# GuildOfWeavers/distaff

Hardware: AMD Instinct MI355X
Metric: trace_cells_per_sec (higher is better)
Workload: dtype u128 (prime field 2^128-45*2^40+1, 4x u32 limbs)

## Files before the change

distaff_amd/csrc/ctx.h:

```cpp
#pragma once
#include <hip/hip_runtime.h>
#include <stdint.h>
#include <string.h>
#include <memory>
#include <string>
#include <map>
#include <vector>
#include "fe.h"
#include "../../include/distaff_hip.h"

struct __attribute__((aligned(16))) digest { uint32_t w[8]; };
#define AIR_PERIODIC_STRIDE 29

#ifndef NTT_TW4_PAIRS
#define NTT_TW4_PAIRS 0
#endif
#if NTT_TW4_PAIRS
typedef fe_tw tw4_t;
#else
typedef fe tw4_t;
#endif

#define DST_MAX_FRI_LAYERS 24

struct dst_switch_def { const char* name; bool product; const char* values; const char* what; };
static const dst_switch_def DST_SWITCHES[] = {
    {"DISTAFF_SHARD_DEBUG",        true,  "1",               "stderr line per tree exchange on rank 0; communicators record the order of their collectives (dst_comm_trace)"},
    {"DISTAFF_SHARD_TREE_GATHER",  true,  "1",               "sharded Merkle trees: all-gather of all boundary nodes + upper levels repeated on every rank (BASELINE north_star's all-gather-only form) instead of the k-range all-to-all"},
    {"DISTAFF_SHARD_NO_OVERLAP",   true,  "1",               "sharded prover: every collective on the context's main stream (no second stream / events) also on a stream-ordered transport"},
    {"DISTAFF_COMM_TIMEOUT_S",     true,  "seconds",         "communicators: limit of every host wait behind a collective (default 60; <= 0: none); on expiry the rank aborts the communicator and returns DST_ERR_COMM (dst_comm_set_timeout changes it per handle)"},
    {"DISTAFF_LOCAL_TRANSPORT",    true,  "blocking",        "in-process transport (dst_comm_init_local, dst_prove_sharded_local): drain every rank's stream around each collective instead of the stream-ordered form (events between the ranks' streams, nothing waited for)"},
    {"DISTAFF_TMP_REGS",           true,  "4..W",            "registers per transform launch = size of the staging array (default: as many as 12 GiB hold, at most W)"},
    {"DISTAFF_AIR",                false, "small|deep|generic", "force a more general constraint-kernel instance set than the trace shape needs (generic = per-operation formulation)"},
    {"DISTAFF_BOUNDARY",           false, "eval",            "boundary combinations by evaluation on the 8n domain (the reference's route) instead of coefficient form"},
    {"DISTAFF_COMBINE",            false, "steps",           "combine_polys / DEEP composition as the reference's sequence of whole-array steps instead of the fused passes"},
    {"DISTAFF_NTT",                false, "pre|3pass|reg|lds", "force a transform plan family"},
    {"DISTAFF_NTT_SHAPE",          false, "a,b",             "three-pass plans: log2 of the first two pass lengths"},
    {"DISTAFF_NTT_ORDER",          false, "0",               "first pass of an extension in coset-slow block order"},
    {"DISTAFF_NTT_WAVES",          false, "4|8",             "force the 512- or 1024-lane instances of the LDS passes"},
    {"DISTAFF_NTT_FIXED",          false, "0",               "use the any-shape instances where a shape-compiled one exists"},
    {"DISTAFF_NTT_DIF",            false, "0|1|2",           "first pass of an extension: coset DIT (0), pre-scale + DIF (1), DIT with last-stage twiddles from global memory (2)"},
    {"DISTAFF_NTT_DEBUG",          false, "1",               "print the occupancy of every transform launch shape once"},
    {"DISTAFF_LDE_BATCH",          false, "cols,cosets",     "registers x cosets per transform launch"},
    {"DISTAFF_FOLD8_DFT",          false, "0",               "8n-coefficient extensions without the fused fold + 8-point step"},
    {"DISTAFF_TRACE_BUFFER",       false, "1",               "give the trace its own buffer instead of coset 0 of the extension"},
    {"DISTAFF_MERKLE_LEVEL2_LOG",  false, "k",               "build two tree levels per launch from 2^k grandparents per launch on (default 2^19)"},
    {"DISTAFF_MERKLE_LEVELS",      false, "1",               "one launch per tree level"},
    {"DISTAFF_SYN_DIV_TABLES",     false, "1",               "synthetic division by power tables + scan instead of the blocked form"},
    {"DISTAFF_FRI_TAIL",           false, "0",               "no single-launch tail: every FRI layer by its own launches (the tail otherwise starts at the first layer of at most 2^13 elements)"},
    {"DISTAFF_FRI_CHAIN",          false, "0",               "FRI commit phase with a root read-back and a host draw per layer"},
    {"DISTAFF_FRI_REPLICATE_LOG",  false, "k",               "sharded prover: replicate FRI layers from 2^k elements on (default 2^17)"},
    {"DISTAFF_SHARD_FORCE_OVERLAP", false, "1",              "sharded prover: the two-stream choreography of a stream-ordered transport over a blocking one"},
    {"DISTAFF_TEST_STALL_COLLECTIVE", false, "k|k@r",        "communicators: fault injection -- before device collective number k (of rank r only) a kernel holds the stream until the communicator is aborted"},
};
enum : size_t {
    HS_WEIGHTS = 0,
    HS_WEIGHTS_BYTES = (4 * 128 + 4) * 16,
    HS_DEEP = 32768,
    HS_DEEP_HALF = 2048,
    HS_FRI_ROOTS = 40960,
    HS_FRI_SLOTS = 45056,
    HS_FRI_SLOT_BYTES = 800,
    HS_AIR_FLAG = 65536 - 64,
    HS_DRAWS = 65536,
    HS_DRAWS_BYTES = (344 + 160) * 16,
    HS_COMPOSE = 65536 + 8192,
    HS_COMPOSE_BYTES = 516 * 16,
    HS_STATUS = 65536 + 8192 + 8320,
    HS_STATUS_SLOTS = 32,
// ... 22 lines not shown
    DST_BUF_TRACE_LEAVES = 2,
    DST_BUF_TRACE_NODES = 3,
    DST_BUF_CEVAL_I = 4,
    DST_BUF_CEVAL_F = 5,
    DST_BUF_CEVAL_T = 6,
    DST_BUF_CPOLY = 7,
    DST_BUF_CEVALS = 8,
    DST_BUF_CNODES = 9,
    DST_BUF_COMP_POLY = 10,
    DST_BUF_COMP_EVALS = 11,
    DST_BUF_FRI_EVALS = 12,
    DST_BUF_FRI_NODES = 13,
    DST_BUF_FRI_LEAVES = 14,
};

struct NttInstance;
struct NttRegInstance;
enum NttKind : uint32_t { NTT_FIRST, NTT_MIDDLE, NTT_LAST };
struct NttPass {
    NttKind kind = NTT_FIRST;
    uint32_t log_len = 0;
    uint32_t log_tile = 0, pre = 0;
    uint32_t dit = 0;
    size_t lds = 0;
    const NttInstance* inst = nullptr;
    const NttRegInstance* reg = nullptr;
    const fe_tw* stage_tw[2] = {nullptr, nullptr}; const fe_tw* pre_tw[2] = {nullptr, nullptr}; const tw4_t* tw4[2] = {nullptr, nullptr};
};
struct NttPlan {
    uint32_t log_n1 = 0, log_n2 = 0;
    uint32_t log_n3 = 0;
    uint32_t count = 0;
    bool coset_slow = false; uint32_t debug = 0;
    NttPass pass[3], first_lde;
    const NttPass& at(uint32_t i, bool lde) const { return (i == 0 && lde) ? first_lde : pass[i]; }
};

struct dst_ctx {
    dst_params prm{};
    std::string err;
    std::map<std::string, std::string> sw_values;
    const char* sw(const char* name) const { auto it = sw_values.find(name); return it == sw_values.end() ? nullptr : it->second.c_str(); }
    bool sw_is(const char* name, const char* value) const { const char* v = sw(name); return v && !strcmp(v, value); }
    bool sw_flag(const char* name) const { const char* v = sw(name); return v && v[0] && v[0] != '0'; }
    void read_switches() {
        sw_values.clear();
        for (const dst_switch_def& d : DST_SWITCHES)
            if (d.product || DST_TEST_HOOKS) if (const char* v = getenv(d.name)) sw_values[d.name] = v;
    }
    int device = 0;
    hipStream_t stream = nullptr;

    uint32_t log_n = 0, log_b = 0, log_N = 0;
    size_t n = 0, B = 0, N = 0, W = 0;
    size_t Bc = 0, j0 = 0;
    size_t stack_depth = 0;
    NttPlan plan;
    std::vector<fe> air_draws;
    std::shared_ptr<void> open_plan;
    std::vector<uint64_t> open_plan_positions;
    uint8_t open_plan_root[32] = {0};
    int fri_rep_from = 0;
    bool fri_tail_pending = false;
    fe* fri_nat0 = nullptr;
    bool sharded_layout = false;

// ... 171 lines not shown
```

distaff_amd/csrc/kernels_ntt.hip:

```cpp
#include "ctx.h"
#include "host/ctx_tables.h"
#include <mutex>
#include <type_traits>
#include "ntt_lds.h"

#if defined(NTT_NO_ROTATE)
#define NTT_NO_ROTATE_DEFINED 1
#else
#define NTT_NO_ROTATE_DEFINED 0
#endif
#define NTT_TILE_ELEMS 4096

struct NttArgs {
    const fe* src; fe* dst;
    size_t src_col_stride, src_coset_stride;
    size_t dst_col_stride, dst_coset_stride;
    const fe_tw* stage_tw;
    const fe_tw* prescale;
    const fe_tw* dit_last;
    const tw4_t* tw4;
    size_t tw4_coset_stride;
    uint32_t log_n1, log_n2, tile , log_N, log_b;
    uint32_t j0;
    uint32_t has_scale;
    uint32_t tiles_per_block;
    uint32_t debug;
    size_t src_row_stride, dst_k_stride, src_batch_stride, dst_batch_stride;
    uint32_t batch_log;
    uint32_t dit;
    uint32_t groups, cosets, cols;
    uint32_t coset_fast;
    uint32_t pre;
    const fe_tw* pre_tw;
    fe_tw scale;
};

__device__ __forceinline__ fe load_fe(const fe* p) { return *p; }

__device__ __forceinline__ fe dom_pow(const fe* lo, const fe* hi, uint32_t lo_bits, uint64_t e) {
    uint32_t l = (uint32_t)e & ((1u << lo_bits) - 1u), h = (uint32_t)(e >> lo_bits);
    fe a = lo[l];
    if (h == 0) return a;
    return fe_mul(a, hi[h]);
}

__device__ __forceinline__ void ntt_block(const NttArgs& a, uint32_t& group, uint32_t& jl, uint32_t& col) {
    const uint32_t b = blockIdx.x, units = a.groups * a.cosets;
    uint32_t u;
    if (a.coset_fast) {
        const uint32_t s = b >> 3, pairs = a.cosets * a.cols, pair = s % pairs;
        group = (s / pairs) * 8u + (b & 7u);
        const uint32_t chunk = pair / (4u * a.cosets), in_chunk = pair - chunk * 4u * a.cosets;
        const uint32_t width = (chunk * 4u + 4u <= a.cols) ? 4u : a.cols - chunk * 4u;
        col = chunk * 4u + in_chunk % width; jl = in_chunk / width;
// ... 42 lines not shown
#if defined(NTT_LAB_STAMPS)
#define NTT_LAB_WG_STRIDE 61u
__device__ unsigned long long ntt_lab_buf[2 * 256 * 16 * 2 * 16];
extern "C" __attribute__((visibility("default"))) int dst_lab_stamps(unsigned long long* out, size_t count, int clear) {
    if (count > sizeof(ntt_lab_buf) / 8) return -1;
    if (hipMemcpyFromSymbol(out, HIP_SYMBOL(ntt_lab_buf), count * 8) != hipSuccess) return -2;
    if (clear) { static unsigned long long zero[2 * 256 * 16 * 2 * 16]; if (hipMemcpyToSymbol(HIP_SYMBOL(ntt_lab_buf), zero, sizeof zero) != hipSuccess) return -3; }
    return 0;
}
#define NTT_LAB_FLUSH(pass, it, st, nst) do { \
    if ((blockIdx.x % NTT_LAB_WG_STRIDE) == 0u && blockIdx.x / NTT_LAB_WG_STRIDE < 256u && (it) < 2u && (threadIdx.x & 63u) == 0u) { \
        unsigned long long* o_ = ntt_lab_buf + ((((size_t)(pass) * 256u + blockIdx.x / NTT_LAB_WG_STRIDE) * 16u + (threadIdx.x >> 6)) * 2u + (it)) * 16u; \
        for (int k_ = 0; k_ < (nst); k_++) o_[k_] = (st)[k_]; } } while (0)
#else
#define NTT_LAB_FLUSH(pass, it, st, nst) ((void)0)
#endif
extern __shared__ __attribute__((aligned(16))) unsigned char ntt_smem[];

template <int THREADS, int WPE = 4, bool PREFETCH = true, int LOG_LEN = 0, int LOG_T = 0, int PRE = 0>
__global__ void __launch_bounds__(THREADS, WPE) ntt_pass_a(NttArgs a, const fe* __restrict__ src_base, fe* __restrict__ dst_base) {
    constexpr int EPT = NTT_TILE_ELEMS / THREADS;
    fe* L = reinterpret_cast<fe*>(ntt_smem);
    const uint32_t log_n1 = LOG_LEN ? (uint32_t)LOG_LEN : a.log_n1;
    const uint32_t log_t = LOG_T ? (uint32_t)LOG_T : a.tile, T = 1u << log_t, n1 = 1u << log_n1;
    fe_tw* TW = reinterpret_cast<fe_tw*>(L + n1 * T);
    uint32_t group, jl, col;
    ntt_block(a, group, jl, col);
    uint32_t hh = 0;
    if (PRE) { const uint32_t half = a.groups >> 1; hh = group >= half ? 1u : 0u; group -= hh * half; }
    const uint32_t jg = a.j0 + jl;
    const fe* __restrict__ src0 = src_base + (size_t)col * a.src_col_stride + (size_t)jl * a.src_coset_stride;
    fe* __restrict__ dst0 = dst_base + (size_t)col * a.dst_col_stride + (size_t)jl * a.dst_coset_stride;
    const uint32_t pmask = (1u << (a.log_b + log_n1 + PRE)) - 1u;
    const uint32_t jv = jg + (hh << a.log_b);
    if (a.dit) {
        const uint32_t in_lds = a.dit_last ? n1 / 2 : n1;
        for (uint32_t i = threadIdx.x; i + 1 < in_lds; i += THREADS) {
            const uint32_t lb = 31u - (uint32_t)__clz(i + 1), k = i + 1 - (1u << lb);
            TW[i] = a.prescale[((jv + (k << (a.log_b + PRE))) << (log_n1 - lb - 1)) & pmask];
        }
    } else
    for (uint32_t i = threadIdx.x; i < n1 / 2; i += THREADS) TW[dif_tw_slot(i)] = a.stage_tw[i];
    const bool scaled = !a.dit && a.prescale != nullptr && jg != 0;
    fe pre0 = fe_zero(), pre1 = fe_zero(), pre2 = fe_zero(), pre3 = fe_zero(), pre4 = fe_zero(), pre5 = fe_zero(), pre6 = fe_zero(), pre7 = fe_zero();
    const uint32_t count = n1 * T;
#define NTT_EACH(M) { M(0, pre0) M(1, pre1) M(2, pre2) M(3, pre3) M(4, pre4) M(5, pre5) M(6, pre6) M(7, pre7) }
    const bool rot_a = a.dit && log_t == 2 && !NTT_NO_ROTATE_DEFINED;
#define NTT_COL_A(idx) (rot_a ? (((idx) + ((idx) >> log_t)) & (T - 1)) : ((idx) & (T - 1)))
    const fe_tw pre_c = (PRE && a.dit) ? a.prescale[(jg << log_n1) & pmask] : fe_tw{};
    auto pre_stage_a = [&](const fe& x0, const fe& x1, uint32_t row) -> fe {
        if (a.dit) { const fe t = fe_mul_tw(x1, pre_c); return hh ? fe_sub(x0, t) : fe_add(x0, t); }
        return hh ? fe_mul_tw(fe_sub(x0, x1), a.pre_tw[row]) : fe_add(x0, x1);
    };
#define NTT_FETCH_A1(e, var) if constexpr ((e) < EPT) { uint32_t idx = lane + (e) * THREADS; idx = idx < count ? idx : 0u; \
        if constexpr (PRE != 0) { const uint32_t row_ = idx >> log_t; const fe x0_ = src[NTT_LAB_SRC(row_, NTT_COL_A(idx), (row_ << a.log_n2) + NTT_COL_A(idx))], x1_ = src[NTT_LAB_SRC(row_ + 512u, NTT_COL_A(idx), ((row_ + n1) << a.log_n2) + NTT_COL_A(idx))]; var = pre_stage_a(x0_, x1_, row_); } \
        else var = src[NTT_LAB_SRC(idx >> log_t, NTT_COL_A(idx), ((idx >> log_t) << a.log_n2) + NTT_COL_A(idx))]; }
#define NTT_FETCH_A(tile) { const fe* __restrict__ src = src0 + (tile) * T; NTT_EACH(NTT_FETCH_A1) }
    const tw4_t* __restrict__ tw4 = a.tw4 + (size_t)jl * a.tw4_coset_stride;
    const uint32_t tile0 = group * a.tiles_per_block;
    uint32_t lane = threadIdx.x;
    if (PREFETCH) NTT_FETCH_A(tile0)
    for (uint32_t it = 0; it < a.tiles_per_block; it++) {
        const uint32_t tile = tile0 + it;
        unsigned long long st[16]; (void)st;
        NTT_STAMP_REAL(st, 14);
        NTT_STAMP(st, 8);
        lane = lds_opaque_lane();
        if (!PREFETCH) NTT_FETCH_A(tile)
        NTT_STAMP(st, 9);
        __syncthreads();
        NTT_STAMP(st, 10);
#define NTT_PUT_A(e, var) if constexpr ((e) < EPT) { const uint32_t idx = lane + (e) * THREADS; if (idx < count) { if (a.dit) L[lds_slot(__brev(idx >> log_t) >> (32 - log_n1), NTT_COL_A(idx), log_t)] = var; else L[lds_slot(idx >> log_t, idx & (T - 1), log_t)] = scaled ? fe_mul_tw(var, a.prescale[(jg * (idx >> log_t)) & pmask]) : var; } }
        NTT_EACH(NTT_PUT_A)
#undef NTT_PUT_A
        NTT_STAMP(st, 11);
        __syncthreads();
        NTT_STAMP(st, 12);
        if (PREFETCH && it + 1 < a.tiles_per_block) NTT_FETCH_A(tile + 1)
        if constexpr (LOG_LEN != 0) {
            if (a.dit) lds_ntt_dit_fixed<THREADS, LOG_LEN, LOG_T>(L, TW, a.dit_last ? a.dit_last + (size_t)((jg << PRE) + hh) * (n1 / 2) : nullptr, NttKeepInLds(), st);
            else lds_ntt_dif_fixed<THREADS, LOG_LEN, LOG_T>(L, TW, NttKeepInLds(), st);
        } else {
            if (a.dit) lds_ntt_dit<THREADS>(L, TW, log_n1, log_t, 1u, log_n1 + 1u, a.dit_last ? a.dit_last + (size_t)((jg << PRE) + hh) * (n1 / 2) : nullptr);
            else lds_ntt_dif<THREADS>(L, TW, log_n1, log_t, 1u, log_n1 + 1u);
        }
        constexpr int RB = WPE > 4 ? 1 : THREADS == 512 ? 2 : 4;
#if defined(NTT_LAB_DST_DENSE)
        fe* __restrict__ dst = dst_base + ((size_t)blockIdx.x * a.tiles_per_block + it) * count;
#else
        fe* __restrict__ dst = dst0 + tile * T;
#endif
        const tw4_t* __restrict__ tw = tw4 + tile * T;
        for (uint32_t base = 0; base < count; base += RB * THREADS) {
            fe v[RB]; tw4_t w[RB]; uint32_t off[RB]; bool ok[RB];
            static_for<0, RB>([&](auto q_) {
                constexpr int q = decltype(q_)::value;
                uint32_t idx = base + q * THREADS + lane;
                ok[q] = idx < count;
                idx = ok[q] ? idx : 0u;
                const uint32_t t = idx & (T - 1), r = idx >> log_t;
                const uint32_t k1 = ((a.dit ? r : __brev(r) >> (32 - log_n1)) << PRE) + hh;
                off[q] = (k1 << a.log_n2) + t;
                v[q] = L[idx];
                w[q] = tw[NTT_LAB_TW(r, t, off[q])];
#if defined(NTT_LAB_DST_DENSE)
                off[q] = idx;
#endif
            });
            static_for<0, RB>([&](auto q_) {
                constexpr int q = decltype(q_)::value;
#if NTT_TW4_PAIRS
                const fe out_q = fe_mul_tw(v[q], w[q]);
#else
                const fe out_q = fe_mul(v[q], w[q]);
#endif
#if NTT_STREAM_STORE
                if (ok[q]) fe_store_stream(dst + off[q], out_q);
#else
                if (ok[q]) dst[off[q]] = out_q;
#endif
            });
        }
        NTT_STAMP(st, 13);
        NTT_STAMP_REAL(st, 15);
        NTT_LAB_FLUSH(0, it, st, 16);
    }
}

template <int THREADS, int WPE = 4, bool PREFETCH = true, int LOG_LEN = 0, int LOG_T = 0, int PRE = 0>
__global__ void __launch_bounds__(THREADS, WPE) ntt_pass_b(NttArgs a, const fe* __restrict__ src_base, fe* __restrict__ dst_base) {
    constexpr int EPT = NTT_TILE_ELEMS / THREADS;
    fe* L = reinterpret_cast<fe*>(ntt_smem);
    const uint32_t log_n2 = LOG_LEN ? (uint32_t)LOG_LEN : a.log_n2;
    const uint32_t log_t = LOG_T ? (uint32_t)LOG_T : a.tile, T = 1u << log_t, n2 = 1u << log_n2;
    fe_tw* TW = reinterpret_cast<fe_tw*>(L + n2 * T);
    uint32_t g, jl, col;
    ntt_block(a, g, jl, col);
    uint32_t hh = 0;
    if (PRE) { const uint32_t half = a.groups >> 1; hh = g >= half ? 1u : 0u; g -= hh * half; }
    const uint32_t batch = g & ((1u << a.batch_log) - 1u), group = g >> a.batch_log;
    const fe* __restrict__ src = src_base + (size_t)col * a.src_col_stride + (size_t)jl * a.src_coset_stride + (size_t)batch * a.src_batch_stride;
    fe* __restrict__ dst = dst_base + (size_t)col * a.dst_col_stride + (size_t)jl * a.dst_coset_stride + (size_t)batch * a.dst_batch_stride;
    for (uint32_t i = threadIdx.x; i < n2 / 2; i += THREADS) TW[dif_tw_slot(i)] = a.stage_tw[i];
    fe pre0 = fe_zero(), pre1 = fe_zero(), pre2 = fe_zero(), pre3 = fe_zero(), pre4 = fe_zero(), pre5 = fe_zero(), pre6 = fe_zero(), pre7 = fe_zero();
    const uint32_t count = n2 * T;
    const bool colfast_b = log_t == 2 && !NTT_NO_ROTATE_DEFINED;
#define NTT_ROW_B(idx) (colfast_b ? ((idx) & (T - 1)) : ((idx) >> log_n2))
#define NTT_M2_B(idx) (colfast_b ? ((idx) >> log_t) : ((idx) & (n2 - 1)))
#if NTT_STREAM_B_LOAD
#define NTT_LOAD_B(p) fe_load_stream(p)
#else
#define NTT_LOAD_B(p) (*(p))
#endif
#define NTT_FETCH_B1(e, var) if constexpr ((e) < EPT) { uint32_t idx = lane + (e) * THREADS; idx = idx < count ? idx : 0u; \
        if constexpr (PRE != 0) { const uint32_t m_ = NTT_M2_B(idx); const fe* p_ = srct + NTT_ROW_B(idx) * row_stride + m_; const fe x0_ = p_[0], x1_ = p_[n2]; \
                                  var = hh ? fe_mul_tw(fe_sub(x0_, x1_), a.pre_tw[m_]) : fe_add(x0_, x1_); } \
        else var = NTT_LOAD_B(srct + (NTT_ROW_B(idx) * row_stride + NTT_M2_B(idx))); }
#define NTT_FETCH_B(tile) { const fe* __restrict__ srct = src + (size_t)((tile) * T) * a.src_row_stride; NTT_EACH(NTT_FETCH_B1) }
    const uint32_t row_stride = (uint32_t)a.src_row_stride;
    const uint32_t tile0 = group * a.tiles_per_block;
    uint32_t lane = threadIdx.x;
    if (PREFETCH) NTT_FETCH_B(tile0)
    for (uint32_t it = 0; it < a.tiles_per_block; it++) {
        const uint32_t k1_0 = (tile0 + it) * T;
        unsigned long long st[16]; (void)st;
        NTT_STAMP_REAL(st, 14);
        NTT_STAMP(st, 8);
        lane = lds_opaque_lane();
        if (!PREFETCH) NTT_FETCH_B(tile0 + it)
        NTT_STAMP(st, 9);
        __syncthreads();
        NTT_STAMP(st, 10);
#define NTT_PUT_B(e, var) if constexpr ((e) < EPT) { const uint32_t idx = lane + (e) * THREADS; if (idx < count) L[lds_slot(NTT_M2_B(idx), NTT_ROW_B(idx), log_t)] = var; }
        NTT_EACH(NTT_PUT_B)
#undef NTT_PUT_B
        NTT_STAMP(st, 11);
        __syncthreads();
        NTT_STAMP(st, 12);
        if (PREFETCH && it + 1 < a.tiles_per_block) NTT_FETCH_B(tile0 + it + 1)
        const OutB out{dst + k1_0, (uint32_t)a.dst_k_stride, log_n2, a.has_scale != 0, a.scale, (uint32_t)PRE, hh};
        const fe_tw* Wuse = TW;
        if constexpr (LOG_LEN != 0) lds_ntt_dif_fixed<THREADS, LOG_LEN, LOG_T, OutB>(L, Wuse, out, st);
        else lds_ntt_dif<THREADS, OutB>(L, Wuse, log_n2, log_t, 1u, log_n2 + 1u, out);
        NTT_STAMP(st, 13);
        NTT_STAMP_REAL(st, 15);
        NTT_LAB_FLUSH(1, it, st, 16);
    }
}

template <int LOGL> struct NttDigits;
template <> struct NttDigits<6>  { static constexpr int r1 = 3, r2 = 3, r3 = 0, log_t = 2; };
// ... 129 lines not shown
                fe v = x[u * R + rho];
                if (a.tw_lo != nullptr) {
                    uint64_t e = ((uint64_t)m2 * (((uint64_t)k << a.log_b) + (a.coset_twiddle ? jg : 0u))) & nmask;
                    if (e != 0) {
                        const uint32_t el = (uint32_t)e & ((1u << a.lo_bits) - 1u), eh = (uint32_t)(e >> a.lo_bits);
                        v = fe_mul_call(v, a.tw_lo[el]);
                        if (eh != 0) v = fe_mul_call(v, a.tw_hi[eh]);
                    }
                }
                if (a.has_scale) v = fe_mul_call(v, a.scale);
                dst[(size_t)k * a.out_stride_k + t] = v;
            });
        });
    }
}

struct NttInstance { bool pass_b; int threads, wpe; bool prefetch; int log_len, log_t, pre; void (*kernel)(NttArgs, const fe*, fe*); };
#define NTT_INSTANCE(PASS_B, KERNEL, ...) {PASS_B, __VA_ARGS__, KERNEL<__VA_ARGS__>}
static const NttInstance NTT_INSTANCES[] = {
    NTT_INSTANCE(false, ntt_pass_a, 512, 4, true, 0, 0, 0),  NTT_INSTANCE(true, ntt_pass_b, 512, 4, true, 0, 0, 0),
    NTT_INSTANCE(false, ntt_pass_a, 1024, 4, true, 0, 0, 0), NTT_INSTANCE(true, ntt_pass_b, 1024, 4, true, 0, 0, 0),
    NTT_INSTANCE(false, ntt_pass_a, 1024, 8, false, 0, 0, 0), NTT_INSTANCE(true, ntt_pass_b, 1024, 8, false, 0, 0, 0),
    NTT_INSTANCE(false, ntt_pass_a, 1024, 8, false, 10, 2, 0), NTT_INSTANCE(true, ntt_pass_b, 1024, 8, true, 10, 2, 0),
    NTT_INSTANCE(false, ntt_pass_a, 1024, 8, false, 8, 4, 0), NTT_INSTANCE(true, ntt_pass_b, 1024, 8, false, 8, 4, 0),
    NTT_INSTANCE(false, ntt_pass_a, 512, 4, true, 8, 4, 0),   NTT_INSTANCE(true, ntt_pass_b, 512, 4, true, 8, 4, 0),
    NTT_INSTANCE(false, ntt_pass_a, 1024, 8, false, 10, 2, 1), NTT_INSTANCE(true, ntt_pass_b, 1024, 8, false, 10, 2, 1),
    NTT_INSTANCE(false, ntt_pass_a, 512, 4, true, 0, 0, 1),   NTT_INSTANCE(true, ntt_pass_b, 512, 4, true, 0, 0, 1),
};
struct NttRegInstance { int log_len, log_t, threads; void (*kernel)(NttRegArgs); };
#define NTT_REG_INSTANCE(L) {L, NttDigits<L>::log_t, (1 << (L + NttDigits<L>::log_t)) / 16, ntt_reg_kernel<L>}
static const NttRegInstance NTT_REG_INSTANCES[] = {NTT_REG_INSTANCE(6), NTT_REG_INSTANCE(7), NTT_REG_INSTANCE(8), NTT_REG_INSTANCE(9), NTT_REG_INSTANCE(10), NTT_REG_INSTANCE(11), NTT_REG_INSTANCE(12)};

struct NttSwitches {
    enum Force { NONE, OTHER, PRE, THREE, REG, LDS } force = NONE;
    unsigned shape_a = 0, shape_b = 0;
    int waves = 0;
    int dif = -1;
    bool any_shape = false, coset_slow = false;
    uint32_t debug = 0;
};
static NttSwitches ntt_switches(const dst_ctx* c) {
    NttSwitches s;
    if (const char* e = c->sw("DISTAFF_NTT")) s.force = !strcmp(e, "pre") ? s.PRE : !strcmp(e, "3pass") ? s.THREE : !strcmp(e, "reg") ? s.REG : !strcmp(e, "lds") ? s.LDS : s.OTHER;
    if (const char* e = c->sw("DISTAFF_NTT_SHAPE")) if (sscanf(e, "%u,%u", &s.shape_a, &s.shape_b) != 2) s.shape_a = s.shape_b = 0;
    if (const char* e = c->sw("DISTAFF_NTT_WAVES")) s.waves = e[0] == '8' ? 8 : 4;
    if (const char* e = c->sw("DISTAFF_NTT_DIF")) s.dif = e[0] == '0' ? 1 : e[0] == '2' ? 2 : 0;
    s.any_shape = c->sw_is("DISTAFF_NTT_FIXED", "0");
    if (const char* e = c->sw("DISTAFF_NTT_ORDER")) s.coset_slow = e[0] == '0';
    if (const char* e = c->sw("DISTAFF_NTT_DEBUG")) s.debug = (uint32_t)atoi(e);
    return s;
}

#define NTT_LDS_TWO_PER_CU (80 * 1024)
static const NttInstance* ntt_select(bool pass_b, uint32_t log_len, uint32_t log_tile, uint32_t pre, size_t lds, const NttSwitches& sw) {
    const bool two = lds <= NTT_LDS_TWO_PER_CU, eight = two && (sw.waves ? sw.waves == 8 : log_len >= 10);
    const bool fixed = log_len == 10 && log_tile == 2 && !sw.any_shape, fixed84 = log_len == 8 && log_tile == 4 && !sw.any_shape;
    const bool wide8 = pre ? fixed : eight, shaped = pre ? fixed : two && ((eight && fixed) || fixed84);
    const int threads = (wide8 || (!pre && !two)) ? 1024 : 512, wpe = wide8 ? 8 : 4, len = shaped ? (int)log_len : 0, t = shaped ? (int)log_tile : 0;
    for (const NttInstance& r : NTT_INSTANCES)
        if (r.pass_b == pass_b && r.threads == threads && r.wpe == wpe && r.log_len == len && r.log_t == t && r.pre == (int)pre) return &r;
    return nullptr;
}
static uint32_t ntt_first_pass_mode(const NttSwitches& sw, size_t n1, size_t tile) {
    if (sw.dif >= 0) return (uint32_t)sw.dif;
    if (n1 * tile * sizeof(fe) + n1 * sizeof(fe_tw) <= NTT_LDS_TWO_PER_CU) return 1;
    if (n1 * tile * sizeof(fe) + (n1 / 2) * sizeof(fe_tw) <= NTT_LDS_TWO_PER_CU) return 2;
    return 0;
}

static NttPlan ntt_plan_derive(uint32_t log_n, const NttSwitches& sw) {
    NttPlan pl;
    const bool force_pre = sw.force == sw.PRE && log_n >= 10 && log_n <= 22;
    const bool pre_plan = force_pre || ((log_n == 21 || log_n == 22) && sw.force == sw.NONE);
    const bool three = !pre_plan && ((log_n >= 21 && sw.force != sw.REG && sw.force != sw.LDS) || (sw.force == sw.THREE && log_n >= 12));
    uint32_t pre_a = 0, pre_b = 0;
    if (three) {
        uint32_t a = (log_n + 2) / 3, b = (log_n - a + 1) / 2;
        if (a > 8) { a = 8; b = 8; }
        const unsigned x = sw.shape_a, y = sw.shape_b;
        if (x >= 4 && y >= 4 && x <= 8 && y <= 8 && x + y + 4 <= log_n && log_n - x - y <= 8) { a = x; b = y; }
        pl.log_n1 = a; pl.log_n2 = log_n - a; pl.log_n3 = log_n - a - b;
    }
    else { pl.log_n1 = (log_n + 1) / 2; pl.log_n2 = log_n / 2; }
    if (pre_plan) { pre_a = (force_pre || pl.log_n1 > 10) ? 1u : 0u; pre_b = (force_pre || pl.log_n2 > 10) ? 1u : 0u; }
    const bool reg_ok = !three && !pre_plan && pl.log_n2 >= 6 && pl.log_n1 <= 12, reg_all = reg_ok && sw.force == sw.REG;
    const bool reg_a = reg_ok && (pl.log_n1 >= 12 || reg_all), reg_b = reg_ok && (pl.log_n2 >= 12 || reg_all);
    auto pass = [&](NttKind kind, uint32_t log_len, uint32_t other_len_log, uint32_t cap, uint32_t pre, bool reg, bool lde) {
        NttPass P;
        uint32_t t = cap;
        while (t > 1 && (((size_t)1 << log_len) * t * sizeof(fe) > 65536 || t > (1u << other_len_log))) t >>= 1;
        P.kind = kind; P.log_len = log_len; P.log_tile = (uint32_t)__builtin_ctz(t); P.pre = pre;
        const size_t len = (size_t)1 << log_len;
        if (lde && !reg) { P.dit = ntt_first_pass_mode(sw, len, t); if (pre && P.dit == 0) P.dit = 2; }
        P.lds = len * t * sizeof(fe) + (P.dit == 1 ? len : len / 2) * sizeof(fe_tw);
        if (reg) { for (const NttRegInstance& r : NTT_REG_INSTANCES) if (r.log_len == (int)log_len) P.reg = &r; }
        else P.inst = ntt_select(kind == NTT_LAST, log_len, P.log_tile, pre, P.lds, sw);
        return P;
    };
    const uint32_t cap = three ? 16 : 4;
    pl.pass[0] = pass(NTT_FIRST, pl.log_n1 - pre_a, pl.log_n2, cap, pre_a, reg_a, false);
    pl.first_lde = pass(NTT_FIRST, pl.log_n1 - pre_a, pl.log_n2, cap, pre_a, reg_a, true);
    if (three) pl.pass[1] = pass(NTT_MIDDLE, pl.log_n2 - pl.log_n3, pl.log_n3, cap, 0, false, false);
    pl.pass[three ? 2 : 1] = three ? pass(NTT_LAST, pl.log_n3, pl.log_n1, cap, 0, false, false) : pass(NTT_LAST, pl.log_n2 - pre_b, pl.log_n1, cap, pre_b, reg_b, false);
    pl.count = three ? 3 : 2; pl.coset_slow = sw.coset_slow; pl.debug = sw.debug;
    return pl;
}
static int ntt_plan_set(dst_ctx* c) {
    NttPlan& pl = c->plan = ntt_plan_derive(c->log_n, ntt_switches(c));
    for (uint32_t i = 0; i < 2 * pl.count; i++)
        if (!pl.at(i % pl.count, i >= pl.count).inst && !pl.at(i % pl.count, i >= pl.count).reg) { c->err = "transform plan: no compiled instance for pass " + std::to_string(i % pl.count); return DST_ERR_STATE; }
    return DST_OK;
}

static uint32_t ntt_tiles_per_block(uint32_t tiles, size_t arrays) {
    uint32_t k = 1;
    while (k < 8 && tiles % (2 * k) == 0 && (size_t)(tiles / (2 * k)) * arrays >= 2048) k *= 2;
    return k;
}
static void ntt_report_occupancy(const char* name, const NttInstance& I, size_t lds) {
    static std::mutex mu;
    static std::map<std::string, bool> seen;
    char key[128]; snprintf(key, sizeof key, "%s/%d/%d/%d/%d/%d/%zu", name, I.threads, I.wpe, I.log_len, I.log_t, I.pre, lds);
    std::lock_guard<std::mutex> lock(mu);
    if (seen[key]) return; seen[key] = true;
    int nb = -1;
    const hipError_t e = hipOccupancyMaxActiveBlocksPerMultiprocessor(&nb, I.kernel, I.threads, lds);
    fprintf(stderr, "[distaff] %s<%d,%d,%d,%d,%d,%d>: %d lanes, %zu B LDS -> %d workgroups per CU (%s)\n", name, I.threads, I.wpe, (int)I.prefetch, I.log_len, I.log_t, I.pre, I.threads, lds, nb, hipGetErrorString(e));
}

struct NttIo { const fe* src; size_t src_col_stride, src_coset_stride; fe* dst; size_t dst_col_stride, dst_coset_stride; };

static void ntt_run_pass(dst_ctx* c, const NttPass& P, const NttIo& io, size_t cosets, size_t cols, bool inverse, bool lde, uint32_t skip, std::string* describe) {
    const NttPlan& p = c->plan;
    const bool first = P.kind == NTT_FIRST, last = P.kind == NTT_LAST;
    const size_t n = c->n, n1 = (size_t)1 << p.log_n1, nrow = (size_t)1 << p.log_n2;
    const char* name = first ? "ntt_pass_a" : last ? "ntt_pass_b" : "ntt_pass_mid";
    const double bytes = 16.0 * n * cols * ((first && lde) ? 1 + cosets : 2 * cosets);
    const uint32_t j0 = lde ? (uint32_t)c->j0 + skip : 0u, has_scale = (last && inverse) ? 1u : 0u;
    char line[384];
    if (P.reg) {
        const NttRegInstance& R = *P.reg;
        NttRegArgs a{};
        a.log_N = c->log_N; a.log_b = c->log_b; a.lo_bits = c->tw_lo_bits; a.j0 = j0; a.coset_twiddle = lde ? 1u : 0u;
        for (int j = 0; j < 8; j++) a.c16[j] = inverse ? c->c16i[j] : c->c16f[j];
        a.src = io.src; a.src_col_stride = io.src_col_stride; a.src_coset_stride = io.src_coset_stride;
        a.dst = io.dst; a.dst_col_stride = io.dst_col_stride; a.dst_coset_stride = io.dst_coset_stride;
        a.scale = c->n_inv; a.has_scale = has_scale; a.stage_tw = P.stage_tw[inverse];
        if (first) {
            a.in_stride_m = nrow; a.in_stride_t = 1; a.out_stride_k = nrow;
            a.tw_lo = inverse ? c->itw_lo : c->tw_lo; a.tw_hi = inverse ? c->itw_hi : c->tw_hi;
            a.prescale = lde ? c->prescale : nullptr;
        } else { a.in_stride_m = 1; a.in_stride_t = nrow; a.out_stride_k = n1; }
        const dim3 g((unsigned)((first ? nrow : n1) >> R.log_t), (unsigned)cosets, (unsigned)cols);
        if (describe) {
            snprintf(line, sizeof line, "%s reg LOGL=%d block=%d grid=%ux%ux%u lds=0 dit=0 pre=0 log_len=%d log_tile=%d tiles_per_block=1 coset_fast=0 has_scale=%u bytes=%.0f mads=0\n",
                     name, R.log_len, R.threads, g.x, g.y, g.z, R.log_len, R.log_t, has_scale, bytes);
            *describe += line; return;
        }
        KScope ks_(c, name, bytes, true);
        hipLaunchKernelGGL(R.kernel, g, dim3(R.threads), 0, c->stream, a);
        return;
    }
    NttArgs a{};
    a.log_N = c->log_N; a.log_b = c->log_b; a.scale = c->n_inv_tw; a.has_scale = has_scale; a.debug = p.debug;
    a.src = io.src; a.src_col_stride = io.src_col_stride; a.src_coset_stride = io.src_coset_stride;
    a.dst = io.dst; a.dst_col_stride = io.dst_col_stride; a.dst_coset_stride = io.dst_coset_stride;
    a.stage_tw = P.stage_tw[inverse]; a.tile = P.log_tile; a.pre = P.pre; a.pre_tw = P.pre_tw[inverse];
    a.log_n1 = p.log_n1; a.log_n2 = p.log_n2;
    size_t units = cosets;
    uint32_t tiles, batch_log = 0;
    if (first) {
        a.log_n1 = P.log_len; a.j0 = j0;
        a.prescale = lde ? c->prescale : nullptr;
        a.dit = P.dit ? 1u : 0u; a.dit_last = P.dit == 2 ? c->dit_last : nullptr;
        a.tw4 = !lde ? P.tw4[inverse] : describe ? nullptr : c->tw4_lde + (size_t)skip * n; a.tw4_coset_stride = lde ? n : 0;
        tiles = (uint32_t)(nrow >> P.log_tile);
    } else if (!last) {
        a.log_n1 = P.log_len; a.log_n2 = p.log_n3; a.tw4 = P.tw4[inverse];
        a.src_coset_stride = a.dst_coset_stride = nrow; units = cosets * n1;
        tiles = (1u << p.log_n3) >> P.log_tile;
    } else {
        a.log_n2 = P.log_len;
        a.src_row_stride = nrow; a.dst_k_stride = n1;
        if (p.log_n3) { batch_log = p.log_n2 - p.log_n3; a.src_batch_stride = (size_t)1 << p.log_n3; a.dst_k_stride = n1 << batch_log; a.dst_batch_stride = n1; }
        a.batch_log = batch_log;
        tiles = (uint32_t)(n1 >> P.log_tile);
    }
    const uint32_t spread = P.pre + batch_log;
    a.tiles_per_block = ntt_tiles_per_block(tiles, (units * cols) << spread);
    const size_t groups = (size_t)(tiles / a.tiles_per_block) << spread;
    a.coset_fast = (first && cosets > 1 && groups % 8 == 0 && !p.coset_slow) ? 1u : 0u;
    a.groups = (uint32_t)groups; a.cosets = (uint32_t)units; a.cols = (uint32_t)cols;
    const uint32_t stages = P.log_len;
    double mults = a.dit ? 0.5 * stages : ((stages & 1u) ? 0.5 * (stages - 1) : (stages >= 2 ? 0.5 * stages - 0.75 : 0.0));
    if (!last) mults += ((first && lde && !a.dit) ? 1.0 : 0.0) + (NTT_TW4_PAIRS ? 1.0 : 21.0 / 18.0); else if (has_scale) mults += 1.0;
    if (P.pre) mults += a.dit ? 1.0 : 0.5;
    const double elements = (double)groups * a.tiles_per_block * ((size_t)1 << a.tile) * ((size_t)1 << stages) * units * cols;
    const NttInstance& I = *P.inst;
    const unsigned grid = (unsigned)(groups * units * cols);
    if (describe) {
        snprintf(line, sizeof line, "%s lds %c<%d,%d,%d,%d,%d,%d> block=%d grid=%u lds=%zu dit=%u pre=%u log_len=%u log_tile=%u tiles_per_block=%u coset_fast=%u has_scale=%u bytes=%.0f mads=%.0f\n",
                 name, I.pass_b ? 'b' : 'a', I.threads, I.wpe, (int)I.prefetch, I.log_len, I.log_t, I.pre, I.threads, grid, P.lds, P.dit, P.pre, P.log_len, P.log_tile,
                 a.tiles_per_block, a.coset_fast, has_scale, bytes, 18.0 * mults * elements);
        *describe += line; return;
    }
    KScope ks_(c, name, bytes, true, 18.0 * mults * elements);
    if (a.debug & 1u) ntt_report_occupancy(name, I, P.lds);
    hipLaunchKernelGGL(I.kernel, dim3(grid), dim3(I.threads), P.lds, c->stream, a, a.src, a.dst);
}

static void ntt_transform(dst_ctx* c, const NttIo& io, size_t cosets, size_t cols, bool inverse, bool lde, uint32_t skip = 0, std::string* describe = nullptr) {
    const NttPlan& p = c->plan;
    fe* const stage[2] = {c->tmp, c->tmp2};
    for (uint32_t i = 0; i < p.count; i++) {
        NttIo s = io;
        if (i > 0) { s.src = stage[i - 1]; s.src_col_stride = c->n * cosets; s.src_coset_stride = c->n; }
        if (i + 1 < p.count) { s.dst = stage[i]; s.dst_col_stride = c->n * cosets; s.dst_coset_stride = c->n; }
        ntt_run_pass(c, p.at(i, lde), s, cosets, cols, inverse, lde, skip, describe);
    }
}

__global__ void twiddle_table_kernel(tw4_t* out, const fe* tw_lo, const fe* tw_hi, uint32_t lo_bits, uint32_t log_n2, uint32_t log_n, uint32_t log_b,
                                     uint32_t log_N, uint32_t j0, uint32_t coset_twiddle) {
    const size_t n = (size_t)1 << log_n;
    size_t i = (size_t)blockIdx.x * blockDim.x + threadIdx.x;
    if (i >= n) return;
    const uint64_t k1 = i >> log_n2, m2 = i & (((size_t)1 << log_n2) - 1);
    const uint64_t jg = coset_twiddle ? j0 + blockIdx.y : 0;
    const uint64_t e = (m2 * ((k1 << log_b) + jg)) & (((uint64_t)1 << log_N) - 1);
#if NTT_TW4_PAIRS
    out[(size_t)blockIdx.y * n + i] = fe_tw_make(dom_pow(tw_lo, tw_hi, lo_bits, e));
#else
    out[(size_t)blockIdx.y * n + i] = dom_pow(tw_lo, tw_hi, lo_bits, e);
#endif
}
int k_ntt_init(dst_ctx* c) {
    int r = ntt_plan_set(c);
    if (r) return r;
    NttPlan& pl = c->plan;
    {
        static std::mutex mu;
        static bool raised[64] = {};
        std::lock_guard<std::mutex> lock(mu);
        if (c->device >= 0 && c->device < 64 && !raised[c->device]) {
            for (const NttInstance& I : NTT_INSTANCES) HIP_TRY(c, hipFuncSetAttribute((const void*)I.kernel, hipFuncAttributeMaxDynamicSharedMemorySize, 160 * 1024));
            raised[c->device] = true;
        }
    }
    {
        const fe w16 = h_root_of_unity(4);
        const std::vector<fe> f = h_powers(w16, 8), b = h_powers(h_inv(w16), 8);
        for (int j = 0; j < 8; j++) { c->c16f[j] = f[j]; c->c16i[j] = b[j]; }
    }
    for (uint32_t i = 0; i < pl.count; i++) {
        NttPass& P = pl.pass[i];
        const fe w = h_root_of_unity(P.log_len), wp = h_root_of_unity(P.log_len + 1);
        for (int inv = 0; inv < 2; inv++) {
            if ((r = dev_upload(c, &c->ntt_stage_tw[i][inv], h_powers_tw(inv ? h_inv(w) : w, (size_t)1 << (P.log_len - 1))))) return r;
            if (P.pre && (r = dev_upload(c, &c->ntt_pre_tw[i][inv], h_powers_tw(inv ? h_inv(wp) : wp, (size_t)1 << P.log_len)))) return r;
            P.stage_tw[inv] = c->ntt_stage_tw[i][inv]; P.pre_tw[inv] = c->ntt_pre_tw[i][inv];
        }
    }
    {
        const std::vector<fe_tw> pre = h_powers_tw(h_root_of_unity(c->log_b + pl.log_n1), (size_t)1 << (c->log_b + pl.log_n1));
        if ((r = dev_upload(c, &c->prescale, pre))) return r;
        const size_t R = (size_t)1 << pl.pass[0].pre, half = (size_t)1 << (pl.pass[0].log_len - 1);
        std::vector<fe_tw> last(c->B * R * half);
        for (size_t j = 0; j < c->B; j++) for (size_t h = 0; h < R; h++) for (size_t k = 0; k < half; k++) last[(j * R + h) * half + k] = pre[j + c->B * (h + R * k)];
        if ((r = dev_upload(c, &c->dit_last, last))) return r;
    }
    if ((r = dev_alloc(c, &c->tw4_lde, c->Bc * c->n))) return r;
    if ((r = dev_alloc(c, &c->tw4_fwd, c->n))) return r;
    if ((r = dev_alloc(c, &c->tw4_inv, c->n))) return r;
    pl.pass[0].tw4[0] = c->tw4_fwd; pl.pass[0].tw4[1] = c->tw4_inv;
    dim3 g((unsigned)((c->n + 255) / 256), (unsigned)c->Bc);
    hipLaunchKernelGGL(twiddle_table_kernel, g, dim3(256), 0, c->stream, c->tw4_lde, c->tw_lo, c->tw_hi, c->tw_lo_bits, pl.log_n2, c->log_n, c->log_b, c->log_N, (uint32_t)c->j0, 1u);
    g.y = 1;
    hipLaunchKernelGGL(twiddle_table_kernel, g, dim3(256), 0, c->stream, c->tw4_fwd, c->tw_lo, c->tw_hi, c->tw_lo_bits, pl.log_n2, c->log_n, c->log_b, c->log_N, 0u, 0u);
    hipLaunchKernelGGL(twiddle_table_kernel, g, dim3(256), 0, c->stream, c->tw4_inv, c->itw_lo, c->itw_hi, c->tw_lo_bits, pl.log_n2, c->log_n, c->log_b, c->log_N, 0u, 0u);
    if (pl.count == 3) {
        if ((r = dev_alloc(c, &c->tw4_row_fwd, (size_t)1 << pl.log_n2))) return r;
        if ((r = dev_alloc(c, &c->tw4_row_inv, (size_t)1 << pl.log_n2))) return r;
        pl.pass[1].tw4[0] = c->tw4_row_fwd; pl.pass[1].tw4[1] = c->tw4_row_inv;
        dim3 gr((unsigned)((((size_t)1 << pl.log_n2) + 255) / 256), 1u);
        hipLaunchKernelGGL(twiddle_table_kernel, gr, dim3(256), 0, c->stream, c->tw4_row_fwd, c->tw_lo, c->tw_hi, c->tw_lo_bits, pl.log_n3, pl.log_n2, c->log_b + pl.log_n1, c->log_N, 0u, 0u);
        hipLaunchKernelGGL(twiddle_table_kernel, gr, dim3(256), 0, c->stream, c->tw4_row_inv, c->itw_lo, c->itw_hi, c->tw_lo_bits, pl.log_n3, pl.log_n2, c->log_b + pl.log_n1, c->log_N, 0u, 0u);
    }
    for (int inv = 0; inv < 2; inv++) { pl.first_lde.stage_tw[inv] = pl.pass[0].stage_tw[inv]; pl.first_lde.pre_tw[inv] = pl.pass[0].pre_tw[inv]; }
    HIP_TRY(c, hipStreamSynchronize(c->stream));
    HIP_TRY(c, hipGetLastError());
    return DST_OK;
}

#if DST_TEST_HOOKS
extern "C" __attribute__((visibility("default"))) int dst_ntt_describe(uint32_t log_n, uint32_t log_blowup, int inverse, int lde, uint32_t cosets, uint32_t cols, uint32_t skip, char* out, size_t cap) {
    if (!out || log_n < 4 || log_n > 24 || log_blowup < 4 || log_blowup > 8 || !cosets || !cols) return DST_ERR_ARG;
    dst_ctx c;
    c.read_switches();
    c.log_n = log_n; c.log_b = log_blowup; c.log_N = log_n + log_blowup;
    c.n = (size_t)1 << log_n; c.B = c.Bc = (size_t)1 << log_blowup; c.N = c.n * c.B;
    if (int r = ntt_plan_set(&c)) return r;
    std::string text;
    ntt_transform(&c, NttIo{}, cosets, cols, inverse != 0, lde != 0, skip, &text);
    if (text.size() + 1 > cap) return DST_ERR_ARG;
    memcpy(out, text.c_str(), text.size() + 1);
    return DST_OK;
}
#endif

static size_t tmp_capacity_arrays(const dst_ctx* c) { return c->Bc * c->tmp_regs; }

void k_intt_columns(dst_ctx* c, const fe* src, size_t src_stride, fe* dst, size_t ncols) {
    size_t cap = tmp_capacity_arrays(c);
    for (size_t done = 0; done < ncols;) {
        size_t cols = ncols - done < cap ? ncols - done : cap;
        ntt_transform(c, {src + done * src_stride, src_stride, 0, dst + done * c->n, c->n, 0}, 1, cols, true, false);
        done += cols;
    }
}
// ... 213 lines not shown
```

Before: 570.5 million.

## Store NTT intermediate and twiddle tables in tile-major order between passes

For two-pass NTT plans with 4-column tiles and no register passes, the first pass now writes its output, and the twiddle tables are built, in a tile-major layout. Each tile's data is then contiguous. The second pass reads contiguous 16-element runs instead of strided rows. The aim is to turn the strided intermediate writes and reads into dense, coalesced accesses. Adds index arithmetic, a plan flag and a 'row' switch to keep the old layout. Pre-stage plans and also adds a pre_a forcing option.

```diff
diff --git a/distaff_amd/csrc/ctx.h b/distaff_amd/csrc/ctx.h
--- a/distaff_amd/csrc/ctx.h
+++ b/distaff_amd/csrc/ctx.h
@@ -34,7 +34,7 @@
     {"DISTAFF_AIR",                false, "small|deep|generic", "force a more general constraint-kernel instance set than the trace shape needs (generic = per-operation formulation)"},
     {"DISTAFF_BOUNDARY",           false, "eval",            "boundary combinations by evaluation on the 8n domain (the reference's route) instead of coefficient form"},
     {"DISTAFF_COMBINE",            false, "steps",           "combine_polys / DEEP composition as the reference's sequence of whole-array steps instead of the fused passes"},
-    {"DISTAFF_NTT",                false, "pre|3pass|reg|lds", "force a transform plan family"},
+    {"DISTAFF_NTT",                false, "pre|pre_a|3pass|reg|lds|row", "force a transform plan family (pre_a: a register pre-stage in the first pass only; row: the default plan with row-major staging array and tables)"},
     {"DISTAFF_NTT_SHAPE",          false, "a,b",             "three-pass plans: log2 of the first two pass lengths"},
     {"DISTAFF_NTT_ORDER",          false, "0",               "first pass of an extension in coset-slow block order"},
     {"DISTAFF_NTT_WAVES",          false, "4|8",             "force the 512- or 1024-lane instances of the LDS passes"},
@@ -123,6 +123,7 @@
     uint32_t log_n3 = 0;
     uint32_t count = 0;
     bool coset_slow = false; uint32_t debug = 0;
+    bool tile_major = false;
     NttPass pass[3], first_lde;
     const NttPass& at(uint32_t i, bool lde) const { return (i == 0 && lde) ? first_lde : pass[i]; }
 };
diff --git a/distaff_amd/csrc/kernels_ntt.hip b/distaff_amd/csrc/kernels_ntt.hip
--- a/distaff_amd/csrc/kernels_ntt.hip
+++ b/distaff_amd/csrc/kernels_ntt.hip
@@ -20,6 +20,7 @@
     const fe_tw* dit_last;
     const tw4_t* tw4;
     size_t tw4_coset_stride;
+    uint32_t tile_major;
     uint32_t log_n1, log_n2, tile , log_N, log_b;
     uint32_t j0;
     uint32_t has_scale;
@@ -128,6 +129,7 @@
     const fe* __restrict__ src0 = src_base + (size_t)col * a.src_col_stride + (size_t)jl * a.src_coset_stride;
     fe* __restrict__ dst0 = dst_base + (size_t)col * a.dst_col_stride + (size_t)jl * a.dst_coset_stride;
     const uint32_t pmask = (1u << (a.log_b + log_n1 + PRE)) - 1u;
+    const bool tile_major = (LOG_T != 0 && LOG_T != 2) ? false : a.tile_major != 0;
     const uint32_t jv = jg + (hh << a.log_b);
     if (a.dit) {
         const uint32_t in_lds = a.dit_last ? n1 / 2 : n1;
@@ -181,12 +183,9 @@
             else lds_ntt_dif<THREADS>(L, TW, log_n1, log_t, 1u, log_n1 + 1u);
         }
         constexpr int RB = WPE > 4 ? 1 : THREADS == 512 ? 2 : 4;
-#if defined(NTT_LAB_DST_DENSE)
-        fe* __restrict__ dst = dst_base + ((size_t)blockIdx.x * a.tiles_per_block + it) * count;
-#else
-        fe* __restrict__ dst = dst0 + tile * T;
-#endif
-        const tw4_t* __restrict__ tw = tw4 + tile * T;
+        const size_t tile_at = tile_major ? (size_t)tile * (count << PRE) : (size_t)tile * T;
+        fe* __restrict__ dst = dst0 + tile_at;
+        const tw4_t* __restrict__ tw = tw4 + tile_at;
         for (uint32_t base = 0; base < count; base += RB * THREADS) {
             fe v[RB]; tw4_t w[RB]; uint32_t off[RB]; bool ok[RB];
             static_for<0, RB>([&](auto q_) {
@@ -195,13 +194,13 @@
                 ok[q] = idx < count;
                 idx = ok[q] ? idx : 0u;
                 const uint32_t t = idx & (T - 1), r = idx >> log_t;
-                const uint32_t k1 = ((a.dit ? r : __brev(r) >> (32 - log_n1)) << PRE) + hh;
-                off[q] = (k1 << a.log_n2) + t;
+                if (tile_major && a.dit && !PRE) off[q] = idx;
+                else {
+                    const uint32_t k1 = ((a.dit ? r : __brev(r) >> (32 - log_n1)) << PRE) + hh;
+                    off[q] = tile_major ? (k1 << log_t) + t : (k1 << a.log_n2) + t;
+                }
                 v[q] = L[idx];
                 w[q] = tw[NTT_LAB_TW(r, t, off[q])];
-#if defined(NTT_LAB_DST_DENSE)
-                off[q] = idx;
-#endif
             });
             static_for<0, RB>([&](auto q_) {
                 constexpr int q = decltype(q_)::value;
@@ -240,19 +239,22 @@
     for (uint32_t i = threadIdx.x; i < n2 / 2; i += THREADS) TW[dif_tw_slot(i)] = a.stage_tw[i];
     fe pre0 = fe_zero(), pre1 = fe_zero(), pre2 = fe_zero(), pre3 = fe_zero(), pre4 = fe_zero(), pre5 = fe_zero(), pre6 = fe_zero(), pre7 = fe_zero();
     const uint32_t count = n2 * T;
+    const bool tile_major = (PRE || (LOG_T != 0 && LOG_T != 2)) ? false : a.tile_major != 0;
+    const uint32_t run_shift = a.log_n1 + 2u;
     const bool colfast_b = log_t == 2 && !NTT_NO_ROTATE_DEFINED;
-#define NTT_ROW_B(idx) (colfast_b ? ((idx) & (T - 1)) : ((idx) >> log_n2))
-#define NTT_M2_B(idx) (colfast_b ? ((idx) >> log_t) : ((idx) & (n2 - 1)))
+#define NTT_ROW_B(idx) (tile_major ? (((idx) >> 2) & 3u) : colfast_b ? ((idx) & (T - 1)) : ((idx) >> log_n2))
+#define NTT_M2_B(idx) (tile_major ? ((((idx) >> 4) << 2) + ((idx) & 3u)) : colfast_b ? ((idx) >> log_t) : ((idx) & (n2 - 1)))
+#define NTT_OFF_B(idx) (tile_major ? ((((idx) >> 4) << run_shift) + ((idx) & 15u)) : (NTT_ROW_B(idx) * row_stride + NTT_M2_B(idx)))
 #if NTT_STREAM_B_LOAD
 #define NTT_LOAD_B(p) fe_load_stream(p)
 #else
 #define NTT_LOAD_B(p) (*(p))
 #endif
 #define NTT_FETCH_B1(e, var) if constexpr ((e) < EPT) { uint32_t idx = lane + (e) * THREADS; idx = idx < count ? idx : 0u; \
-        if constexpr (PRE != 0) { const uint32_t m_ = NTT_M2_B(idx); const fe* p_ = srct + NTT_ROW_B(idx) * row_stride + m_; const fe x0_ = p_[0], x1_ = p_[n2]; \
+        if constexpr (PRE != 0) { const uint32_t m_ = NTT_M2_B(idx); const fe* p_ = srct + NTT_OFF_B(idx); const fe x0_ = p_[0], x1_ = p_[n2]; \
                                   var = hh ? fe_mul_tw(fe_sub(x0_, x1_), a.pre_tw[m_]) : fe_add(x0_, x1_); } \
-        else var = NTT_LOAD_B(srct + (NTT_ROW_B(idx) * row_stride + NTT_M2_B(idx))); }
-#define NTT_FETCH_B(tile) { const fe* __restrict__ srct = src + (size_t)((tile) * T) * a.src_row_stride; NTT_EACH(NTT_FETCH_B1) }
+        else var = NTT_LOAD_B(srct + NTT_OFF_B(idx)); }
+#define NTT_FETCH_B(tile) { const fe* __restrict__ srct = src + (tile_major ? (size_t)(tile) * (T * T) : (size_t)((tile) * T) * a.src_row_stride); NTT_EACH(NTT_FETCH_B1) }
     const uint32_t row_stride = (uint32_t)a.src_row_stride;
     const uint32_t tile0 = group * a.tiles_per_block;
     uint32_t lane = threadIdx.x;
@@ -448,16 +450,18 @@
 static const NttRegInstance NTT_REG_INSTANCES[] = {NTT_REG_INSTANCE(6), NTT_REG_INSTANCE(7), NTT_REG_INSTANCE(8), NTT_REG_INSTANCE(9), NTT_REG_INSTANCE(10), NTT_REG_INSTANCE(11), NTT_REG_INSTANCE(12)};
 
 struct NttSwitches {
-    enum Force { NONE, OTHER, PRE, THREE, REG, LDS } force = NONE;
+    enum Force { NONE, OTHER, PRE, PRE_A, THREE, REG, LDS } force = NONE;
     unsigned shape_a = 0, shape_b = 0;
     int waves = 0;
     int dif = -1;
     bool any_shape = false, coset_slow = false;
+    bool row_major = false;
     uint32_t debug = 0;
 };
 static NttSwitches ntt_switches(const dst_ctx* c) {
     NttSwitches s;
-    if (const char* e = c->sw("DISTAFF_NTT")) s.force = !strcmp(e, "pre") ? s.PRE : !strcmp(e, "3pass") ? s.THREE : !strcmp(e, "reg") ? s.REG : !strcmp(e, "lds") ? s.LDS : s.OTHER;
+    if (c->sw_is("DISTAFF_NTT", "row")) s.row_major = true;
+    else if (const char* e = c->sw("DISTAFF_NTT")) s.force = !strcmp(e, "pre") ? s.PRE : !strcmp(e, "pre_a") ? s.PRE_A : !strcmp(e, "3pass") ? s.THREE : !strcmp(e, "reg") ? s.REG : !strcmp(e, "lds") ? s.LDS : s.OTHER;
     if (const char* e = c->sw("DISTAFF_NTT_SHAPE")) if (sscanf(e, "%u,%u", &s.shape_a, &s.shape_b) != 2) s.shape_a = s.shape_b = 0;
     if (const char* e = c->sw("DISTAFF_NTT_WAVES")) s.waves = e[0] == '8' ? 8 : 4;
     if (const char* e = c->sw("DISTAFF_NTT_DIF")) s.dif = e[0] == '0' ? 1 : e[0] == '2' ? 2 : 0;
@@ -484,10 +488,15 @@
     return 0;
 }
 
+static bool ntt_tile_major(const NttPlan& pl) {
+    return pl.count == 2 && !pl.pass[0].reg && !pl.first_lde.reg && !pl.pass[1].reg && pl.pass[0].log_tile == 2 && pl.first_lde.log_tile == 2 && pl.pass[1].log_tile == 2
+           && !pl.pass[1].pre;
+}
 static NttPlan ntt_plan_derive(uint32_t log_n, const NttSwitches& sw) {
     NttPlan pl;
     const bool force_pre = sw.force == sw.PRE && log_n >= 10 && log_n <= 22;
-    const bool pre_plan = force_pre || ((log_n == 21 || log_n == 22) && sw.force == sw.NONE);
+    const bool force_pre_a = sw.force == sw.PRE_A && log_n >= 10 && log_n <= 21;
+    const bool pre_plan = force_pre || force_pre_a || ((log_n == 21 || log_n == 22) && sw.force == sw.NONE);
     const bool three = !pre_plan && ((log_n >= 21 && sw.force != sw.REG && sw.force != sw.LDS) || (sw.force == sw.THREE && log_n >= 12));
     uint32_t pre_a = 0, pre_b = 0;
     if (three) {
@@ -498,7 +507,7 @@
         pl.log_n1 = a; pl.log_n2 = log_n - a; pl.log_n3 = log_n - a - b;
     }
     else { pl.log_n1 = (log_n + 1) / 2; pl.log_n2 = log_n / 2; }
-    if (pre_plan) { pre_a = (force_pre || pl.log_n1 > 10) ? 1u : 0u; pre_b = (force_pre || pl.log_n2 > 10) ? 1u : 0u; }
+    if (pre_plan) { pre_a = (force_pre || force_pre_a || pl.log_n1 > 10) ? 1u : 0u; pre_b = (force_pre || pl.log_n2 > 10) ? 1u : 0u; }
     const bool reg_ok = !three && !pre_plan && pl.log_n2 >= 6 && pl.log_n1 <= 12, reg_all = reg_ok && sw.force == sw.REG;
     const bool reg_a = reg_ok && (pl.log_n1 >= 12 || reg_all), reg_b = reg_ok && (pl.log_n2 >= 12 || reg_all);
     auto pass = [&](NttKind kind, uint32_t log_len, uint32_t other_len_log, uint32_t cap, uint32_t pre, bool reg, bool lde) {
@@ -519,6 +528,7 @@
     if (three) pl.pass[1] = pass(NTT_MIDDLE, pl.log_n2 - pl.log_n3, pl.log_n3, cap, 0, false, false);
     pl.pass[three ? 2 : 1] = three ? pass(NTT_LAST, pl.log_n3, pl.log_n1, cap, 0, false, false) : pass(NTT_LAST, pl.log_n2 - pre_b, pl.log_n1, cap, pre_b, reg_b, false);
     pl.count = three ? 3 : 2; pl.coset_slow = sw.coset_slow; pl.debug = sw.debug;
+    pl.tile_major = ntt_tile_major(pl) && !sw.row_major;
     return pl;
 }
 static int ntt_plan_set(dst_ctx* c) {
@@ -583,6 +593,7 @@
     a.dst = io.dst; a.dst_col_stride = io.dst_col_stride; a.dst_coset_stride = io.dst_coset_stride;
     a.stage_tw = P.stage_tw[inverse]; a.tile = P.log_tile; a.pre = P.pre; a.pre_tw = P.pre_tw[inverse];
     a.log_n1 = p.log_n1; a.log_n2 = p.log_n2;
+    a.tile_major = p.tile_major ? 1u : 0u;
     size_t units = cosets;
     uint32_t tiles, batch_log = 0;
     if (first) {
@@ -637,11 +648,13 @@
 }
 
 __global__ void twiddle_table_kernel(tw4_t* out, const fe* tw_lo, const fe* tw_hi, uint32_t lo_bits, uint32_t log_n2, uint32_t log_n, uint32_t log_b,
-                                     uint32_t log_N, uint32_t j0, uint32_t coset_twiddle) {
+                                     uint32_t log_N, uint32_t j0, uint32_t coset_twiddle, uint32_t tile_major) {
     const size_t n = (size_t)1 << log_n;
     size_t i = (size_t)blockIdx.x * blockDim.x + threadIdx.x;
     if (i >= n) return;
-    const uint64_t k1 = i >> log_n2, m2 = i & (((size_t)1 << log_n2) - 1);
+    const uint32_t log_n1 = log_n - log_n2;
+    const uint64_t k1 = tile_major ? (i >> 2) & (((size_t)1 << log_n1) - 1) : i >> log_n2;
+    const uint64_t m2 = tile_major ? ((i >> (log_n1 + 2)) << 2) + (i & 3) : i & (((size_t)1 << log_n2) - 1);
     const uint64_t jg = coset_twiddle ? j0 + blockIdx.y : 0;
     const uint64_t e = (m2 * ((k1 << log_b) + jg)) & (((uint64_t)1 << log_N) - 1);
 #if NTT_TW4_PAIRS
@@ -690,17 +703,18 @@
     if ((r = dev_alloc(c, &c->tw4_inv, c->n))) return r;
     pl.pass[0].tw4[0] = c->tw4_fwd; pl.pass[0].tw4[1] = c->tw4_inv;
     dim3 g((unsigned)((c->n + 255) / 256), (unsigned)c->Bc);
-    hipLaunchKernelGGL(twiddle_table_kernel, g, dim3(256), 0, c->stream, c->tw4_lde, c->tw_lo, c->tw_hi, c->tw_lo_bits, pl.log_n2, c->log_n, c->log_b, c->log_N, (uint32_t)c->j0, 1u);
+    const uint32_t tm = pl.tile_major ? 1u : 0u;
+    hipLaunchKernelGGL(twiddle_table_kernel, g, dim3(256), 0, c->stream, c->tw4_lde, c->tw_lo, c->tw_hi, c->tw_lo_bits, pl.log_n2, c->log_n, c->log_b, c->log_N, (uint32_t)c->j0, 1u, tm);
     g.y = 1;
-    hipLaunchKernelGGL(twiddle_table_kernel, g, dim3(256), 0, c->stream, c->tw4_fwd, c->tw_lo, c->tw_hi, c->tw_lo_bits, pl.log_n2, c->log_n, c->log_b, c->log_N, 0u, 0u);
-    hipLaunchKernelGGL(twiddle_table_kernel, g, dim3(256), 0, c->stream, c->tw4_inv, c->itw_lo, c->itw_hi, c->tw_lo_bits, pl.log_n2, c->log_n, c->log_b, c->log_N, 0u, 0u);
+    hipLaunchKernelGGL(twiddle_table_kernel, g, dim3(256), 0, c->stream, c->tw4_fwd, c->tw_lo, c->tw_hi, c->tw_lo_bits, pl.log_n2, c->log_n, c->log_b, c->log_N, 0u, 0u, tm);
+    hipLaunchKernelGGL(twiddle_table_kernel, g, dim3(256), 0, c->stream, c->tw4_inv, c->itw_lo, c->itw_hi, c->tw_lo_bits, pl.log_n2, c->log_n, c->log_b, c->log_N, 0u, 0u, tm);
     if (pl.count == 3) {
         if ((r = dev_alloc(c, &c->tw4_row_fwd, (size_t)1 << pl.log_n2))) return r;
         if ((r = dev_alloc(c, &c->tw4_row_inv, (size_t)1 << pl.log_n2))) return r;
         pl.pass[1].tw4[0] = c->tw4_row_fwd; pl.pass[1].tw4[1] = c->tw4_row_inv;
         dim3 gr((unsigned)((((size_t)1 << pl.log_n2) + 255) / 256), 1u);
-        hipLaunchKernelGGL(twiddle_table_kernel, gr, dim3(256), 0, c->stream, c->tw4_row_fwd, c->tw_lo, c->tw_hi, c->tw_lo_bits, pl.log_n3, pl.log_n2, c->log_b + pl.log_n1, c->log_N, 0u, 0u);
-        hipLaunchKernelGGL(twiddle_table_kernel, gr, dim3(256), 0, c->stream, c->tw4_row_inv, c->itw_lo, c->itw_hi, c->tw_lo_bits, pl.log_n3, pl.log_n2, c->log_b + pl.log_n1, c->log_N, 0u, 0u);
+        hipLaunchKernelGGL(twiddle_table_kernel, gr, dim3(256), 0, c->stream, c->tw4_row_fwd, c->tw_lo, c->tw_hi, c->tw_lo_bits, pl.log_n3, pl.log_n2, c->log_b + pl.log_n1, c->log_N, 0u, 0u, 0u);
+        hipLaunchKernelGGL(twiddle_table_kernel, gr, dim3(256), 0, c->stream, c->tw4_row_inv, c->itw_lo, c->itw_hi, c->tw_lo_bits, pl.log_n3, pl.log_n2, c->log_b + pl.log_n1, c->log_N, 0u, 0u, 0u);
     }
     for (int inv = 0; inv < 2; inv++) { pl.first_lde.stage_tw[inv] = pl.pass[0].stage_tw[inv]; pl.first_lde.pre_tw[inv] = pl.pass[0].pre_tw[inv]; }
     HIP_TRY(c, hipStreamSynchronize(c->stream));
```

After: 586.0 million (median of 6 runs). 2.7% higher.
